# lainy/sdrangel

Measured on AMD Instinct MI355X. Metric: MS/s complex int16 IQ through decim-64 + DownChannelizer, 1/2/4/8 GPU; % HBM roofline, higher is better.
Workload: dtype int32

## Files before the change

sdrangel_amd/csrc/chan_lower.cpp:

```cpp
#include "chan_lower.hpp"
#include "chan_plan.hpp"
#include <algorithm>

namespace sdrx {

bool subtree_all_mx(const TkSubtree& st)
{
    if (st.n_levels < 1 || st.n_levels > MX_MAX_LEVELS) return false;
    for (int l = 0; l < st.n_levels; l++) if (!st.lv[l].mfma) return false;
    return true;
}

namespace {

std::string lower_job(const TkMJob& j, int PI, int PO, TkLJob& r)
{
    r.b = j.bI; r.c = j.mode ? j.cQ : j.cI; r.out0 = j.out0;
    if (j.bQ != j.bI + PI) return "lower: odd arms not one pitch apart";
    if ((j.mode ? j.cI - j.cQ : j.cQ - j.cI) != PI) return "lower: even arms not one pitch apart";
    bool sink = false;
    int meta = 0;
    for (int k = 0; k < 2; k++) {
        const TkMOut& m = j.o[k];
        const int f = m.flags;
        r.sink[k] = m.sink;
        sink |= m.sink >= 0;
        if (f != 0 && f != (1 | 2) && f != (1 | 4) && f != (1 | 2 | 4)) return "lower: unexpected arm set";
        r.o[k] = f ? m.E_I : 0;
        if (f) {
            if (m.E_Q != m.E_I + PO) return "lower: even arms of a child not one pitch apart";
            const int odd_I = (f & 2) || j.fast ? m.O_I : m.A_I, odd_Q = (f & 2) || j.fast ? m.O_Q : m.A_Q;
            if (odd_I != m.E_I + 2 * PO || odd_Q != m.E_I + 3 * PO) return "lower: odd arm of a child not at 2 pitches";
            if (f == 7 && (m.A_I != m.E_I + 4 * PO || m.A_Q != m.E_I + 5 * PO)) return "lower: alternating arm of a child not at 4 pitches";
        }
        meta |= f << (4 + 4 * k);
    }
    if (!j.mode && (j.o[1].flags || j.o[1].sink >= 0)) return "lower: centre stage with a second child";
    if (j.fast && sink) return "lower: branch-free job with a sink";
    const int cls = j.fast ? MX_FAST : sink ? MX_SINK : MX_ARMS;
    if (j.mode) meta |= MX_LU_BIT;
    r.meta = meta | cls;
    return {};
}

std::string lower_subtree(const BankPlan& plan, const TkSubtree& st, LoweredBank& out)
{
    std::string err;
    for (int l = 0; l < st.n_levels; l++) {
        const TkLevel& lv = st.lv[l];
        const int PI = mx_pitch(l), PO = mx_pitch(l + 1);
        if (lv.in_len * 4 != PI || (lv.arr_cnt && lv.arr_len * 4 != PO)) return "lower: level arrays of another length";
        std::vector<std::pair<int, int>> order;
        std::vector<TkLJob> lowered((size_t)lv.n_mjobs);
        for (int q = 0; q < lv.n_mjobs; q++) {
            const int i = lv.mjob_base + q;
            err = lower_job(plan.mjobs[(size_t)i], PI, PO, lowered[(size_t)q]);
            if (!err.empty()) return err;
            order.emplace_back(mx_class(lowered[(size_t)q].meta), q);
        }
        std::stable_sort(order.begin(), order.end(), [](const std::pair<int, int>& a, const std::pair<int, int>& b) { return a.first < b.first; });
        for (int q = 0; q < lv.n_mjobs; q++) {
            out.jobs[(size_t)(lv.mjob_base + q)] = lowered[(size_t)order[(size_t)q].second];
            out.src[(size_t)(lv.mjob_base + q)] = lv.mjob_base + order[(size_t)q].second;
        }
    }
    return {};
}

}

std::string lower_bank(const BankPlan& plan, LoweredBank& out)
{
    out = LoweredBank{};
    out.jobs.resize(plan.mjobs.size());
    out.src.resize(plan.mjobs.size());
    for (size_t i = 0; i < plan.mjobs.size(); i++) out.src[i] = (int)i;
    std::string first_err;
    std::vector<uint8_t> sub_mx(plan.subtrees.size(), 0);
    for (size_t s = 0; s < plan.subtrees.size(); s++) {
        const TkSubtree& st = plan.subtrees[s];
        if (!plan.mfma || !subtree_all_mx(st)) continue;
        const std::string err = lower_subtree(plan, st, out);
        if (err.empty()) sub_mx[s] = 1;
        else if (first_err.empty()) first_err = err;
    }
    out.pass_mx.assign(plan.passes.size(), 0);
    for (size_t p = 0; p < plan.passes.size(); p++) {
        bool all = !plan.passes[p].empty();
        for (int si : plan.passes[p]) {
            const int s = plan.streams[(size_t)si].subtree;
            all = all && s >= 0 && sub_mx[(size_t)s];
        }
        out.pass_mx[p] = plan.mfma && all ? 1 : 0;
    }
    return first_err;
}

}
```

sdrangel_amd/csrc/chan_lower.hpp:

```cpp
#pragma once
#include "tree_layout.hpp"
#include "hb_consts.hpp"
#include <string>
#include <vector>

namespace sdrx {

struct BankPlan;

constexpr int MX_MAX_LEVELS = 4;

constexpr int mx_pitch(int rel) { return 4 * (HIST / 2 + (TK_CHUNK >> (rel + 2))); }

enum : int {
    MX_FAST = 0,
    MX_ARMS = 1,
    MX_SINK = 2,
    MX_CLASSES = 3
};
constexpr int MX_LU_BIT = 1 << 16;

struct TkLJob {
    int b;
    int c;
    int o[2];
    int sink[2];
    int out0;
    int meta;
};
static_assert(sizeof(TkLJob) == 32, "one s_load_dwordx8 per job");

inline int mx_class(int meta) { return meta & 15; }
inline int mx_flags(int meta, int k) { return (meta >> (4 + 4 * k)) & 15; }

struct LoweredBank {
    std::vector<TkLJob> jobs;
    std::vector<int> src;
    std::vector<uint8_t> pass_mx;
};

bool subtree_all_mx(const TkSubtree& st);

std::string lower_bank(const BankPlan& plan, LoweredBank& out);

}
```

sdrangel_amd/csrc/sdrx_chan.hip:

```cpp
#include "sdrx_common.hpp"
#include "chan_plan.hpp"
#include "tree_kernel.hpp"
#include "tree_mx_kernel.hpp"
#include <vector>
#include <cstring>
#include <new>
#include <algorithm>
#include "chan_plan.cpp"
#include "chan_lower.cpp"

using namespace sdrx;

namespace {

struct Channel {
    int32_t out_rate = 0, ofs = 0;
    int n = 0;
    uint8_t modes[32] = { 0 };
    int group = -1;
    bool passthrough = false;
    bool dead = false;
    DevBuf out;
    int64_t avail = 0;
    int64_t last_off = 0, last_n = 0;
};

struct StreamBuf {
    uint32_t* hist[2] = { nullptr, nullptr };
    int cur = 0;
    DevBuf mid;
};

struct Group {
    int index = -1;
    int64_t T = 0;
    std::vector<int> chans;
    BankPlan plan;
    LoweredBank low;
    std::vector<StreamBuf> bufs;
    void* d_static = nullptr;
    TkSubtree* d_subtrees = nullptr; TkNode* d_nodes = nullptr; TkArray* d_arrays = nullptr; TkMJob* d_mjobs = nullptr;
    TkLJob* d_ljobs = nullptr;
};

}

struct sdrx_chan_bank {
    int device = 0, cus = 256;
    int32_t in_rate = 0;
    hipStream_t own_stream = nullptr, stream = nullptr;
    std::vector<Channel> ch;
    std::vector<Group*> groups;
    DevBuf stage_in;
    DevBuf scratch;
    static constexpr int RING = 4;
    void* h_dyn[RING] = { nullptr, nullptr, nullptr, nullptr };
    void* d_dyn[RING] = { nullptr, nullptr, nullptr, nullptr };
    size_t dyn_cap[RING] = { 0, 0, 0, 0 };
    hipEvent_t dyn_ev[RING] = { nullptr, nullptr, nullptr, nullptr };
    int dyn_next = 0;
    char last_name[96] = "";
    int last_grid = 0, last_block = 0, last_lds = 0;
    EventTimer timer;
};

static void free_group(Group* g)
{
    if (!g) return;
    for (auto& s : g->bufs) { for (uint32_t* h : s.hist) if (h) (void)hipFree(h); s.mid.release(); }
    if (g->d_static) (void)hipFree(g->d_static);
    delete g;
}

static int upload_group(sdrx_chan_bank* b, Group* g)
{
    const BankPlan& p = g->plan;
    g->bufs.resize(p.streams.size());
    for (size_t si = 0; si < p.streams.size(); si++) {
        const size_t bytes = (size_t)p.streams[si].hist_len * 4;
        for (uint32_t*& h : g->bufs[si].hist) {
            SDRX_HIP(hipMalloc(reinterpret_cast<void**>(&h), bytes));
            SDRX_HIP(hipMemsetAsync(h, 0, bytes, b->stream));
        }
    }
    const size_t b0 = p.subtrees.size() * sizeof(TkSubtree), b1 = p.nodes.size() * sizeof(TkNode), b2 = p.arrays.size() * sizeof(TkArray);
    const size_t b3 = p.mjobs.size() * sizeof(TkMJob), b4 = g->low.jobs.size() * sizeof(TkLJob);
    if (b0 + b1 + b2 == 0) return SDRX_OK;
    SDRX_HIP(hipMalloc(&g->d_static, b0 + b1 + b2 + b3 + b4 + 64));
    char* d = static_cast<char*>(g->d_static);
    g->d_subtrees = reinterpret_cast<TkSubtree*>(d);
    g->d_nodes = reinterpret_cast<TkNode*>(d + b0);
    g->d_arrays = reinterpret_cast<TkArray*>(d + b0 + b1);
    g->d_mjobs = reinterpret_cast<TkMJob*>(d + b0 + b1 + b2);
    g->d_ljobs = reinterpret_cast<TkLJob*>(d + b0 + b1 + b2 + b3);
    if (b0) SDRX_HIP(hipMemcpy(g->d_subtrees, p.subtrees.data(), b0, hipMemcpyHostToDevice));
    if (b1) SDRX_HIP(hipMemcpy(g->d_nodes, p.nodes.data(), b1, hipMemcpyHostToDevice));
    if (b2) SDRX_HIP(hipMemcpy(g->d_arrays, p.arrays.data(), b2, hipMemcpyHostToDevice));
    if (b3) SDRX_HIP(hipMemcpy(g->d_mjobs, p.mjobs.data(), b3, hipMemcpyHostToDevice));
    if (b4) SDRX_HIP(hipMemcpy(g->d_ljobs, g->low.jobs.data(), b4, hipMemcpyHostToDevice));
    return SDRX_OK;
}

static int configure_channel(sdrx_chan_bank* b, int c, int32_t req_rate, int32_t req_fc)
{
    Channel& ch = b->ch[c];
    ch.n = plan_chain(b->in_rate, req_rate, req_fc, ch.modes, MAX_STAGES, &ch.out_rate, &ch.ofs);
    ch.passthrough = ch.n == 0;
    return SDRX_OK;
}

static int new_group(sdrx_chan_bank* b, const std::vector<int>& chans)
{
    if (chans.empty()) return SDRX_OK;
    std::vector<PlanChain> chains;
    for (int c : chans) chains.push_back(PlanChain{ c, b->ch[(size_t)c].n, b->ch[(size_t)c].modes });
    BankPlan plan;
    const std::string err = plan_bank(chains, plan_options_from_env(), plan);
    if (!err.empty()) { set_error(err); return SDRX_EINVAL; }
    LoweredBank low;
    (void)lower_bank(plan, low);
    Group* g = new (std::nothrow) Group;
    if (!g) return SDRX_ENOMEM;
    g->chans = chans;
    g->index = (int)b->groups.size();
    g->plan = std::move(plan);
    g->low = std::move(low);
    int rc = upload_group(b, g);
    if (rc) { free_group(g); return rc; }
    for (int c : chans) b->ch[c].group = g->index;
    b->groups.push_back(g);
    return SDRX_OK;
}

static int retire_dead_groups(sdrx_chan_bank* b)
{
    for (size_t gi = 0; gi < b->groups.size();) {
        Group* g = b->groups[gi];
        bool live = false;
        for (int c : g->chans) if (b->ch[(size_t)c].group == g->index) { live = true; break; }
        if (live) { gi++; continue; }
        SDRX_HIP(hipStreamSynchronize(b->stream));
        free_group(g);
        b->groups.erase(b->groups.begin() + (long)gi);
        for (size_t k = gi; k < b->groups.size(); k++) {
            const int old = b->groups[k]->index;
            b->groups[k]->index = (int)k;
            for (int c : b->groups[k]->chans) if (b->ch[(size_t)c].group == old) b->ch[(size_t)c].group = (int)k;
        }
    }
    return SDRX_OK;
}

static int grow_keep(sdrx_chan_bank* b, DevBuf& buf, size_t used, size_t need)
{
    if (need <= buf.cap) return SDRX_OK;
    size_t want = buf.cap ? buf.cap : (1 << 16);
    while (want < need) want *= 2;
    void* np = nullptr;
    SDRX_HIP(hipMalloc(&np, want));
    if (used) SDRX_HIP(hipMemcpyAsync(np, buf.p, used, hipMemcpyDeviceToDevice, b->stream));
    SDRX_HIP(hipStreamSynchronize(b->stream));
    if (buf.p) (void)hipFree(buf.p);
    buf.p = np; buf.cap = want;
    return SDRX_OK;
}

static int dyn_slot(sdrx_chan_bank* b, size_t bytes, int* slot)
{
    const int s = b->dyn_next; b->dyn_next = (b->dyn_next + 1) % sdrx_chan_bank::RING;
    if (b->dyn_ev[s]) SDRX_HIP(hipEventSynchronize(b->dyn_ev[s]));
    else SDRX_HIP(hipEventCreateWithFlags(&b->dyn_ev[s], hipEventDisableTiming));
    if (bytes > b->dyn_cap[s]) {
        size_t want = b->dyn_cap[s] ? b->dyn_cap[s] : 4096; while (want < bytes) want *= 2;
        if (b->h_dyn[s]) (void)hipHostFree(b->h_dyn[s]);
        if (b->d_dyn[s]) (void)hipFree(b->d_dyn[s]);
        b->h_dyn[s] = b->d_dyn[s] = nullptr; b->dyn_cap[s] = 0;
        SDRX_HIP(hipHostMalloc(&b->h_dyn[s], want, hipHostMallocDefault));
        SDRX_HIP(hipMalloc(&b->d_dyn[s], want));
        b->dyn_cap[s] = want;
    }
    *slot = s;
    return SDRX_OK;
}

static int feed_group(sdrx_chan_bank* b, Group* g, const uint32_t* d_in, int64_t n)
{
    const int64_t T0 = g->T, T1 = g->T + n;
    for (int c : g->chans) {
        Channel& ch = b->ch[c];
        if (ch.group != g->index) continue;
        const int64_t add = (T1 >> ch.n) - (T0 >> ch.n);
        int rc = grow_keep(b, ch.out, (size_t)ch.avail * 4, (size_t)(ch.avail + add) * 4 + 64); if (rc) return rc;
    }
    const BankPlan& plan = g->plan;
    for (size_t si = 1; si < plan.streams.size(); si++) {
        const int64_t add = (T1 >> plan.streams[si].depth) - (T0 >> plan.streams[si].depth);
        int rc = g->bufs[si].mid.reserve((size_t)add * 4 + 64); if (rc) return rc;
    }
    const size_t ns = plan.streams.size(), nk = plan.sinks.size();
    const size_t o_sinks = ns * sizeof(TkStream), o_hist = o_sinks + nk * sizeof(TkSink), total = o_hist + ns * sizeof(TkHistJob);
    int slot; int rc = dyn_slot(b, total, &slot); if (rc) return rc;
    char* hp = static_cast<char*>(b->h_dyn[slot]); char* dp = static_cast<char*>(b->d_dyn[slot]);
    TkStream* hs = reinterpret_cast<TkStream*>(hp);
    TkSink* hk = reinterpret_cast<TkSink*>(hp + o_sinks);
    TkHistJob* hh = reinterpret_cast<TkHistJob*>(hp + o_hist);

    std::vector<long> segs(ns, 0);
    for (size_t si = 0; si < ns; si++) {
        const PlanStream& s = plan.streams[si];
        const StreamBuf& sb = g->bufs[si];
        TkStream& t = hs[si];
        t.hist = sb.hist[sb.cur];
        t.in = si == 0 ? d_in : static_cast<const uint32_t*>(sb.mid.p);
        t.t_old = T0 >> s.depth; t.t_new = T1 >> s.depth;
        t.subtree = s.subtree;
        t.c_first = t.t_old / TK_CHUNK;
        t.c_last = t.t_new > t.t_old ? (t.t_new - 1) / TK_CHUNK : t.c_first - 1;
        t.cps = 1;
        t.hist_len = s.hist_len;
        hh[si] = TkHistJob{ sb.hist[sb.cur], t.in, sb.hist[sb.cur ^ 1], t.t_new - t.t_old, s.hist_len };
    }
    for (size_t k = 0; k < nk; k++) {
        const PlanSink& si = plan.sinks[k];
        TkSink& t = hk[k];
        t.shift = 0; t.next = si.next;
        if (si.kind == 0) {
            Channel& ch = b->ch[si.ch];
            t.lo = T0 >> si.depth; t.hi = T1 >> si.depth;
            t.ptr0 = reinterpret_cast<uint32_t*>(reinterpret_cast<uintptr_t>(ch.out.p) - (uintptr_t)(4 * (t.lo - ch.avail)));
            t.shift = si.depth;
            if (ch.group != g->index) t.hi = t.lo;
        } else {
            const int depth = plan.streams[(size_t)si.stream].depth;
            t.lo = T0 >> depth; t.hi = T1 >> depth;
            t.ptr0 = reinterpret_cast<uint32_t*>(reinterpret_cast<uintptr_t>(g->bufs[(size_t)si.stream].mid.p) - (uintptr_t)(4 * t.lo));
        }
    }
    for (const std::vector<int>& ps : plan.passes) {
        long total_chunks = 0;
        for (int si : ps) total_chunks += std::max(0L, hs[si].c_last - hs[si].c_first + 1);
        long cps = (total_chunks + (long)b->cus * 4 - 1) / ((long)b->cus * 4);
        cps = std::max(1L, std::min(cps, 256L));
        for (int si : ps) {
            hs[si].cps = (int)cps;
            segs[si] = (std::max(0L, hs[si].c_last - hs[si].c_first + 1) + cps - 1) / cps;
        }
    }
    SDRX_HIP(hipMemcpyAsync(dp, hp, total, hipMemcpyHostToDevice, b->stream));
    SDRX_HIP(hipEventRecord(b->dyn_ev[slot], b->stream));

    const TkStream* d_streams = reinterpret_cast<const TkStream*>(dp);
    const TkSink* d_sinks = reinterpret_cast<const TkSink*>(dp + o_sinks);
    const TkHistJob* d_hist = reinterpret_cast<const TkHistJob*>(dp + o_hist);
    rc = b->timer.begin(b->stream); if (rc) return rc;
    for (size_t p = 0; p < plan.passes.size(); p++) {
        const std::vector<int>& ps = plan.passes[p];
        if (ps.empty()) continue;
        long max_segs = 0;
        for (int si : ps) max_segs = std::max(max_segs, segs[si]);
        if (max_segs == 0) continue;
        const int s0 = ps.front(), cnt = (int)ps.size();
        size_t lds_bytes = 0;
        for (int si : ps) lds_bytes = std::max(lds_bytes, (size_t)plan.subtrees[(size_t)plan.streams[(size_t)si].subtree].lds_dwords * 4);
        if (g->low.pass_mx[p])
            hipLaunchKernelGGL(tree_mx_kernel, dim3((unsigned)max_segs, (unsigned)cnt), dim3(TK_THREADS), lds_bytes, b->stream,
                               g->d_subtrees, g->d_arrays, d_streams + s0, d_sinks, g->d_ljobs);
        else if (plan.mfma)
            hipLaunchKernelGGL(tree_kernel<true>, dim3((unsigned)max_segs, (unsigned)cnt), dim3(TK_THREADS), lds_bytes, b->stream,
                               g->d_subtrees, g->d_nodes, g->d_arrays, d_streams + s0, d_sinks, g->d_mjobs);
        else
            hipLaunchKernelGGL(tree_kernel<false>, dim3((unsigned)max_segs, (unsigned)cnt), dim3(TK_THREADS), lds_bytes, b->stream,
                               g->d_subtrees, g->d_nodes, g->d_arrays, d_streams + s0, d_sinks, g->d_mjobs);
        SDRX_HIP(hipGetLastError());
        if (p == 0) {
            snprintf(b->last_name, sizeof b->last_name, plan.mfma ? "tree_kernel<mfma>" : "tree_kernel<valu>");
            b->last_grid = (int)(max_segs * cnt); b->last_block = TK_THREADS; b->last_lds = (int)lds_bytes;
        }
    }
    rc = b->timer.end(b->stream); if (rc) return rc;
    long max_hist = TK_HIST;
    for (const PlanStream& s : plan.streams) max_hist = std::max(max_hist, s.hist_len);
    hipLaunchKernelGGL(tree_hist_kernel, dim3((unsigned)(max_hist / 256), (unsigned)ns), dim3(256), 0, b->stream, d_hist);
    SDRX_HIP(hipGetLastError());
    for (StreamBuf& sb : g->bufs) sb.cur ^= 1;
    for (int c : g->chans) {
        Channel& ch = b->ch[c];
        if (ch.group != g->index) continue;
        const int64_t add = (T1 >> ch.n) - (T0 >> ch.n);
        ch.last_off = ch.avail; ch.last_n = add; ch.avail += add;
    }
    g->T = T1;
    return SDRX_OK;
}

static int feed_passthrough(sdrx_chan_bank* b, const uint32_t* d_in, int64_t n)
{
    for (auto& ch : b->ch) {
        if (!ch.passthrough) continue;
        int rc = grow_keep(b, ch.out, (size_t)ch.avail * 4, (size_t)(ch.avail + n) * 4 + 64); if (rc) return rc;
        SDRX_HIP(hipMemcpyAsync(static_cast<uint32_t*>(ch.out.p) + ch.avail, d_in, (size_t)n * 4, hipMemcpyDeviceToDevice, b->stream));
        ch.last_off = ch.avail; ch.last_n = n; ch.avail += n;
    }
    return SDRX_OK;
}

extern "C" {

int sdrx_chan_plan(int32_t in_rate, int32_t req_rate, int32_t req_fc, uint8_t* modes, int32_t* out_rate, int32_t* residual_ofs)
{
    if (!modes || !out_rate || !residual_ofs) { set_error("sdrx_chan_plan: null argument"); return SDRX_EINVAL; }
    return plan_chain(in_rate, req_rate, req_fc, modes, MAX_STAGES, out_rate, residual_ofs);
}

int sdrx_chan_bank_create(sdrx_chan_bank_t** out, int device, int32_t in_rate, int32_t n_ch,
                          const int32_t* req_rate, const int32_t* req_fc)
{
    if (!out) { set_error("sdrx_chan_bank_create: null out"); return SDRX_EINVAL; }
    *out = nullptr;
    if (n_ch <= 0 || !req_rate || !req_fc || in_rate <= 0) { set_error("sdrx_chan_bank_create: bad argument"); return SDRX_EINVAL; }
    int rc = check_device(device); if (rc) return rc;
    SDRX_HIP(hipSetDevice(device));
    sdrx_chan_bank* b = new (std::nothrow) sdrx_chan_bank;
    if (!b) return SDRX_ENOMEM;
    b->device = device; b->in_rate = in_rate; b->cus = device_cu_count(device);
    hipError_t e = hipStreamCreateWithFlags(&b->own_stream, hipStreamNonBlocking);
    if (e != hipSuccess) { delete b; return hip_fail(e, "hipStreamCreate", __FILE__, __LINE__); }
    b->stream = b->own_stream;
    e = hipFuncSetAttribute(reinterpret_cast<const void*>(&tree_kernel<true>), hipFuncAttributeMaxDynamicSharedMemorySize, 160 * 1024);
    if (e == hipSuccess) e = hipFuncSetAttribute(reinterpret_cast<const void*>(&tree_kernel<false>), hipFuncAttributeMaxDynamicSharedMemorySize, 160 * 1024);
    if (e == hipSuccess) e = hipFuncSetAttribute(reinterpret_cast<const void*>(&tree_mx_kernel), hipFuncAttributeMaxDynamicSharedMemorySize, 160 * 1024);
    if (e != hipSuccess) { sdrx_chan_bank_destroy(b); return hip_fail(e, "hipFuncSetAttribute", __FILE__, __LINE__); }
    b->ch.resize((size_t)n_ch);
    std::vector<int> all;
    for (int c = 0; c < n_ch; c++) {
        configure_channel(b, c, req_rate[c], req_fc[c]);
        if (!b->ch[c].passthrough) all.push_back(c);
    }
    rc = new_group(b, all);
    if (rc) { sdrx_chan_bank_destroy(b); return rc; }
    SDRX_HIP(hipStreamSynchronize(b->stream));
    *out = b;
    return SDRX_OK;
}

int sdrx_chan_bank_destroy(sdrx_chan_bank_t* b)
{
    if (!b) return SDRX_OK;
    (void)hipSetDevice(b->device);
    if (b->stream) (void)hipStreamSynchronize(b->stream);
    for (Group* g : b->groups) free_group(g);
    for (auto& c : b->ch) c.out.release();
    b->stage_in.release(); b->scratch.release(); b->timer.release();
    for (int i = 0; i < sdrx_chan_bank::RING; i++) {
        if (b->h_dyn[i]) (void)hipHostFree(b->h_dyn[i]);
        if (b->d_dyn[i]) (void)hipFree(b->d_dyn[i]);
        if (b->dyn_ev[i]) (void)hipEventDestroy(b->dyn_ev[i]);
    }
    if (b->own_stream) (void)hipStreamDestroy(b->own_stream);
    delete b;
    return SDRX_OK;
}

int sdrx_chan_bank_info(const sdrx_chan_bank_t* b, int32_t c, int32_t* n_stages, uint8_t* modes, int32_t* out_rate, int32_t* residual_ofs)
{
    if (!b || c < 0 || c >= (int32_t)b->ch.size()) { set_error("sdrx_chan_bank_info: bad channel"); return SDRX_EINVAL; }
    const Channel& ch = b->ch[(size_t)c];
    if (n_stages) *n_stages = ch.n;
    if (modes) memcpy(modes, ch.modes, (size_t)ch.n);
    if (out_rate) *out_rate = ch.out_rate;
    if (residual_ofs) *residual_ofs = ch.ofs;
    return SDRX_OK;
}

int sdrx_chan_bank_reconfigure(sdrx_chan_bank_t* b, int32_t c, int32_t req_rate, int32_t req_fc)
{
    if (!b || c < 0 || c >= (int32_t)b->ch.size()) { set_error("sdrx_chan_bank_reconfigure: bad channel"); return SDRX_EINVAL; }
    SDRX_HIP(hipSetDevice(b->device));
    Channel& ch = b->ch[(size_t)c];
    ch.group = -1; ch.dead = false;
    configure_channel(b, c, req_rate, req_fc);
    int rc = retire_dead_groups(b); if (rc) return rc;
    if (ch.passthrough) return SDRX_OK;
    return new_group(b, std::vector<int>{ (int)c });
}

int sdrx_chan_bank_add_channel(sdrx_chan_bank_t* b, int32_t req_rate, int32_t req_fc, int32_t* channel)
{
    if (!b) { set_error("sdrx_chan_bank_add_channel: null bank"); return SDRX_EINVAL; }
    SDRX_HIP(hipSetDevice(b->device));
    b->ch.emplace_back();
    const int c = (int)b->ch.size() - 1;
    configure_channel(b, c, req_rate, req_fc);
    if (channel) *channel = c;
    if (b->ch[(size_t)c].passthrough) return SDRX_OK;
    const int rc = new_group(b, std::vector<int>{ c });
    if (rc) { b->ch.pop_back(); if (channel) *channel = -1; }
    return rc;
}

int sdrx_chan_bank_remove_channel(sdrx_chan_bank_t* b, int32_t c)
{
    if (!b || c < 0 || c >= (int32_t)b->ch.size()) { set_error("sdrx_chan_bank_remove_channel: bad channel"); return SDRX_EINVAL; }
    SDRX_HIP(hipSetDevice(b->device));
    Channel& ch = b->ch[(size_t)c];
    ch.group = -1; ch.passthrough = false; ch.dead = true; ch.n = 0; ch.out_rate = 0; ch.ofs = 0;
    ch.avail = 0; ch.last_off = 0; ch.last_n = 0;
    return retire_dead_groups(b);
}

static const int64_t CHAN_STATE_MAGIC = 0x7364727863686b31LL;

int64_t sdrx_chan_bank_state_bytes(const sdrx_chan_bank_t* b)
{
    if (!b) return SDRX_EINVAL;
    int64_t n = 16;
    for (const Group* g : b->groups) { n += 16; for (const PlanStream& s : g->plan.streams) n += 8 + (int64_t)s.hist_len * 4; }
    return n;
}

// ... 199 lines not shown
```

sdrangel_amd/csrc/tree_mx_kernel.hpp:

```cpp
#pragma once
#include "hb_common.hpp"
#include "hb_mfma.hpp"
#include "tree_layout.hpp"
#include "chan_lower.hpp"

namespace sdrx {

__device__ __forceinline__ int mx_div_pow2_trunc(int v, int n)
{
    return (v + ((v >> 31) & ((1 << n) - 1))) >> n;
}

__global__ __launch_bounds__(TK_THREADS, 4)
void tree_mx_kernel(const TkSubtree* __restrict__ subtrees, const TkArray* __restrict__ arrays, const TkStream* __restrict__ streams,
                    const TkSink* __restrict__ sinks, const TkLJob* __restrict__ ljobs)
{
    constexpr int C = TK_CHUNK, NT = TK_THREADS, LPT = C / 4 / NT;
    extern __shared__ __attribute__((aligned(16))) uint32_t lds[];

    const TkStream sp = streams[blockIdx.y];
    const long first = sp.c_first + (long)blockIdx.x * sp.cps;
    if (first > sp.c_last) return;
    long last = first + sp.cps - 1; if (last > sp.c_last) last = sp.c_last;
    const TkSubtree& st = subtrees[sp.subtree];
    const int tid = threadIdx.x;

    for (int i = tid; i < st.lds_dwords; i += NT) lds[i] = 0;
    __syncthreads();
    for (int i = tid; i < st.n_arrays * 16; i += NT) {
        const TkArray a = arrays[st.array_base + (i >> 4)];
        if (a.bias) lds[a.store + (i & 15)] = HBM_BIAS2;
    }
    typedef HbMfmaTaps<48, false> Taps;
    Taps taps;
    const int lane = tid & 63, n16 = lane & 15, g4 = lane >> 4;
    const int wv = __builtin_amdgcn_readfirstlane(tid >> 6);
    taps.init(lane);
    const uint32_t root_xm = st.root_xm;
    int n_levels = st.n_levels, store_base = st.store_base, root_off = st.root_off, root_len = st.root_len;
    asm volatile("" : "+s"(n_levels), "+s"(store_base), "+s"(root_off), "+s"(root_len));
    int rE_I = st.rootE_I, rE_Q = st.rootE_Q, rO_I = st.rootO_I, rO_Q = st.rootO_Q, rA_I = st.rootA_I, rA_Q = st.rootA_Q, root_cnt16 = st.root_arr_cnt * 16;
    asm volatile("" : "+s"(rE_I), "+s"(rE_Q), "+s"(rO_I), "+s"(rO_Q), "+s"(rA_I), "+s"(rA_Q), "+s"(root_cnt16));

    uint4 pre[LPT];
    auto fetch = [&](long chunk, const int tid) {
        const long c0 = chunk * C;
        if (c0 >= sp.t_old && c0 + C <= sp.t_new) {
            typedef uint32_t u4v __attribute__((ext_vector_type(4)));
            typedef const u4v __attribute__((address_space(1))) gq4;
            gq4* src = (gq4*)reinterpret_cast<const u4v*>(sp.in + (c0 - sp.t_old));
#pragma unroll
            for (int j = 0; j < LPT; j++) { const u4v v = src[j * NT + tid]; pre[j] = make_uint4(v[0], v[1], v[2], v[3]); }
            return;
        }
#pragma unroll
        for (int j = 0; j < LPT; j++) {
            const long p0 = chunk * C + 4 * (j * NT + tid);
            if (p0 >= sp.t_old && p0 + 4 <= sp.t_new) {
                pre[j] = *reinterpret_cast<const uint4*>(sp.in + (p0 - sp.t_old));
            } else {
                uint32_t v[4];
#pragma unroll
                for (int e = 0; e < 4; e++) {
                    const long p = p0 + e;
                    v[e] = p < sp.t_old ? sp.hist[p - (sp.t_old - sp.hist_len)] : (p < sp.t_new ? sp.in[p - sp.t_old] : 0u);
                }
                pre[j] = make_uint4(v[0], v[1], v[2], v[3]);
            }
        }
        __builtin_amdgcn_s_waitcnt(0x0F70);
    };
    fetch(first - st.warm, tid);
    __syncthreads();

    typedef int s8i __attribute__((ext_vector_type(8)));
    typedef int s16i __attribute__((ext_vector_type(16)));
    typedef unsigned short us2 __attribute__((ext_vector_type(2)));
    const v4i bias = { Taps::BIAS, Taps::BIAS, Taps::BIAS, Taps::BIAS };
    const char* ldsb = reinterpret_cast<const char*>(lds);
    char* ldsw = reinterpret_cast<char*>(lds);
    const int wl = 32 * n16 + 16 * g4, cl = 32 * n16 + 8 * g4, pl = 16 * n16 + 4 * g4;
    constexpr uint32_t PLAIN = 0x00010001u, ALT = 0x0001ffffu;
    auto padd = [](uint32_t a, uint32_t b) { return __builtin_bit_cast(uint32_t, (us2)(__builtin_bit_cast(us2, a) + __builtin_bit_cast(us2, b))); };
    auto psub = [](uint32_t a, uint32_t b) { return __builtin_bit_cast(uint32_t, (us2)(__builtin_bit_cast(us2, a) - __builtin_bit_cast(us2, b))); };
    auto pmul = [](uint32_t a, uint32_t m) { return __builtin_bit_cast(uint32_t, (us2)(__builtin_bit_cast(us2, a) * __builtin_bit_cast(us2, m))); };

    for (long chunk = first - st.warm; chunk <= last; ++chunk) {
        int tid = threadIdx.x;
        asm volatile("" : "+v"(tid));
#pragma unroll
        for (int j = 0; j < LPT; j++) {
            const int q = HIST / 2 + j * NT + tid;
            const uint4 v = pre[j];
            const uint32_t oI = __builtin_amdgcn_perm(v.w, v.y, 0x05040100u);
            const uint32_t oQ = __builtin_amdgcn_perm(v.w, v.y, 0x07060302u);
            lds[rE_I + q] = __builtin_amdgcn_perm(v.z, v.x, 0x05040100u);
            lds[rE_Q + q] = __builtin_amdgcn_perm(v.z, v.x, 0x07060302u);
            if (rO_I >= 0) { lds[rO_I + q] = oI ^ root_xm; lds[rO_Q + q] = oQ ^ root_xm; }
            if (rA_I >= 0) { lds[rA_I + q] = pmul(oI, ALT) ^ root_xm; lds[rA_Q + q] = pmul(oQ, ALT) ^ root_xm; }
        }
        for (int i = tid; i < root_cnt16; i += NT)
            lds[root_off + (i >> 4) * root_len + (i & 15)] = lds[store_base + i];
        if (chunk < last) fetch(chunk + 1, tid);
        __syncthreads();

        const bool live = chunk >= first;
        int lv0 = 0;
        asm volatile("" : "+s"(lv0), "+s"(n_levels));
        auto level = [&](auto Lc) {
            constexpr int L = decltype(Lc)::value;
            constexpr int PI = mx_pitch(L), PO = mx_pitch(L + 1);
            const s16i rec = *(const s16i __attribute__((address_space(4)))*)reinterpret_cast<const int*>(&st.lv[L + lv0]);
            const int nout = rec[3], arr_base = rec[4], arr_cnt = rec[5], in_len = rec[7], mjob_base = rec[9], n_mjobs = rec[10];
            const uint32_t xm = (uint32_t)rec[11];
            const int prev_off = rec[12], prev_arr_cnt = rec[13], arr_off = rec[14], arr_len = rec[15];
            {
                const int n_restore = arr_cnt * 16, n_all = n_restore + prev_arr_cnt * 16;
                const int slot0 = store_base + 16 * arr_base;
                for (int i = tid; i < n_all; i += NT) {
                    const int k = i - n_restore;
                    const int src = k < 0 ? slot0 + i : prev_off + (k >> 4) * in_len + in_len - 16 + (k & 15);
                    const int dst = k < 0 ? arr_off + (i >> 4) * arr_len + (i & 15) : slot0 - prev_arr_cnt * 16 + k;
                    lds[dst] = lds[src];
                }
            }
            struct JobIn { v4i bI0, bI1, bQ0, bQ1; uint2 cI01, cQ01; uint32_t cI2, cQ2; };
            auto load = [&](const s8i d, JobIn& r, auto Cc) {
                const char* pb = ldsb + d[0] + wl;
                r.bI0 = *reinterpret_cast<const v4i*>(__builtin_assume_aligned(pb, 16));
                r.bI1 = *reinterpret_cast<const v4i*>(__builtin_assume_aligned(pb + 64, 16));
                r.bQ0 = *reinterpret_cast<const v4i*>(__builtin_assume_aligned(pb + PI, 16));
                r.bQ1 = *reinterpret_cast<const v4i*>(__builtin_assume_aligned(pb + PI + 64, 16));
                const char* pc = ldsb + d[1] + cl;
                const char *pI, *pQ;
                if constexpr (decltype(Cc)::value == MX_FAST) { pI = pc + PI; pQ = pc; }
                else { const bool lu = d[7] & MX_LU_BIT; pI = lu ? pc + PI : pc; pQ = lu ? pc : pc + PI; }
                r.cI01 = *reinterpret_cast<const uint2*>(__builtin_assume_aligned(pI, 8));
                r.cI2 = *reinterpret_cast<const uint32_t*>(pI + 8);
                r.cQ01 = *reinterpret_cast<const uint2*>(__builtin_assume_aligned(pQ, 8));
                r.cQ2 = *reinterpret_cast<const uint32_t*>(pQ + 8);
            };
            auto st32 = [&](char* p, int off, uint32_t v) { *reinterpret_cast<uint32_t*>(p + off) = v; };
            auto child = [&](auto Sk, const uint32_t eI, const uint32_t oI, const uint32_t eQ, const uint32_t oQ, const int base, const int f,
                             const int sink, const long abs0) {
                constexpr bool SINK = decltype(Sk)::value;
                if (f) {
                    char* p = ldsw + base + pl;
                    const uint32_t m = (f & 2) ? PLAIN : ALT;
                    st32(p, 0, eI); st32(p, PO, eQ);
                    st32(p, 2 * PO, pmul(oI, m) ^ xm); st32(p, 3 * PO, pmul(oQ, m) ^ xm);
                    if (f == 7) { st32(p, 4 * PO, pmul(oI, ALT) ^ xm); st32(p, 5 * PO, pmul(oQ, ALT) ^ xm); }
                }
                if constexpr (SINK) {
                    if (live) {
                        typedef const s8i __attribute__((address_space(4))) cs8;
                        for (int si = sink; si >= 0; ) {
                            const s8i sr = *(cs8*)reinterpret_cast<const int*>(sinks + si);
                            const long ptr0 = ((long)sr[1] << 32) | (uint32_t)sr[0];
                            const long lo = ((long)sr[3] << 32) | (uint32_t)sr[2], hi = ((long)sr[5] << 32) | (uint32_t)sr[4];
                            const int shift = sr[6];
                            uint32_t w[4];
                            if (shift) {
                                w[0] = pack_iq(mx_div_pow2_trunc((int)(int16_t)eI, shift), mx_div_pow2_trunc((int)(int16_t)eQ, shift));
                                w[1] = pack_iq(mx_div_pow2_trunc((int)(int16_t)oI, shift), mx_div_pow2_trunc((int)(int16_t)oQ, shift));
                                w[2] = pack_iq(mx_div_pow2_trunc((int)eI >> 16, shift), mx_div_pow2_trunc((int)eQ >> 16, shift));
                                w[3] = pack_iq(mx_div_pow2_trunc((int)oI >> 16, shift), mx_div_pow2_trunc((int)oQ >> 16, shift));
                            } else {
                                w[0] = __builtin_amdgcn_perm(eQ, eI, 0x05040100u); w[1] = __builtin_amdgcn_perm(oQ, oI, 0x05040100u);
                                w[2] = __builtin_amdgcn_perm(eQ, eI, 0x07060302u); w[3] = __builtin_amdgcn_perm(oQ, oI, 0x07060302u);
                            }
                            typedef uint32_t __attribute__((address_space(1))) gu32;
                            gu32* dst = (gu32*)(reinterpret_cast<uint32_t*>(ptr0) + abs0);
                            const long rel = abs0 - lo, span = hi - lo;
                            if (rel >= 0 && rel + 4 <= span) {
                                typedef uint32_t u4a __attribute__((ext_vector_type(4), aligned(4)));
                                *(u4a __attribute__((address_space(1)))*)dst = u4a{ w[0], w[1], w[2], w[3] };
                            } else if (rel > -4 && rel < span) {
#pragma unroll
                                for (int i = 0; i < 4; i++) if (rel + i >= 0 && rel + i < span) dst[i] = w[i];
                            }
                            si = sr[7];
                        }
                    }
                }
            };
            auto finish = [&](auto Cc, const JobIn& r, const v4i SI, const v4i SQ, const s8i d) {
                constexpr int CLS = decltype(Cc)::value;
                auto shpack = [](int a, int b) {
                    uint32_t v = (uint32_t)(a >> (HB_SHIFT - 1));
                    asm("v_ashrrev_i32_sdwa %0, %1, %2 dst_sel:WORD_1 dst_unused:UNUSED_PRESERVE src0_sel:DWORD src1_sel:DWORD" : "+v"(v) : "s"(HB_SHIFT - 1), "v"(b));
                    return v;
                };
                const uint32_t sI02 = shpack(SI[0], SI[2]), sI13 = shpack(SI[1], SI[3]);
                const uint32_t sQ02 = shpack(SQ[0], SQ[2]), sQ13 = shpack(SQ[1], SQ[3]);
                const uint32_t cI02 = __builtin_amdgcn_perm(r.cI01.y, r.cI01.x, 0x07060302u), cI13 = __builtin_amdgcn_perm(r.cI2, r.cI01.y, 0x05040100u);
                const uint32_t cQ02 = __builtin_amdgcn_perm(r.cQ01.y, r.cQ01.x, 0x07060302u), cQ13 = __builtin_amdgcn_perm(r.cQ2, r.cQ01.y, 0x05040100u);
                const int meta = d[7], f0 = (meta >> 4) & 15, f1 = (meta >> 8) & 15;
                if constexpr (CLS == MX_FAST) {
                    const uint32_t ma = (f0 & 2) ? PLAIN : ALT, mb = (f1 & 2) ? PLAIN : ALT;
                    auto st4 = [&](const int base, uint32_t eI, uint32_t eQ, uint32_t oI, uint32_t oQ, uint32_t m) {
                        char* p = ldsw + base + pl;
                        st32(p, 0, eI); st32(p, PO, eQ); st32(p, 2 * PO, pmul(oI, m) ^ xm); st32(p, 3 * PO, pmul(oQ, m) ^ xm);
                    };
                    st4(d[2], padd(sI02, cI02), psub(sQ02, cQ02), psub(sI13, cI13), padd(sQ13, cQ13), ma);
                    st4(d[3], psub(sI02, cI02), padd(sQ02, cQ02), padd(sI13, cI13), psub(sQ13, cQ13), mb);
                } else {
                    const std::integral_constant<bool, CLS == MX_SINK> Sk;
                    const long abs0 = CLS == MX_SINK ? chunk * nout + d[6] + 16 * n16 + 4 * g4 : 0;
                    const uint32_t sg = (meta & MX_LU_BIT) ? 0xffffffffu : PLAIN;
                    if (f0 | (d[4] >= 0)) {
                        const uint32_t nI13 = pmul(cI13, sg), nQ02 = pmul(cQ02, sg);
                        child(Sk, padd(sI02, cI02), padd(sI13, nI13), padd(sQ02, nQ02), padd(sQ13, cQ13), d[2], f0, d[4], abs0);
                    }
                    if (f1 | (d[5] >= 0)) child(Sk, psub(sI02, cI02), padd(sI13, cI13), padd(sQ02, cQ02), psub(sQ13, cQ13), d[3], f1, d[5], abs0);
                }
            };
            auto pair = [&](auto Cc, const s8i d0, const s8i d1) {
                JobIn r0, r1;
                __builtin_amdgcn_s_setprio(2);
                load(d0, r0, Cc); load(d1, r1, Cc);
                __builtin_amdgcn_sched_barrier(0);
                const v4i SI0 = taps.tile(r0.bI0, r0.bI1, bias), SQ0 = taps.tile(r0.bQ0, r0.bQ1, bias);
                const v4i SI1 = taps.tile(r1.bI0, r1.bI1, bias), SQ1 = taps.tile(r1.bQ0, r1.bQ1, bias);
                __builtin_amdgcn_s_setprio(0);
                finish(Cc, r0, SI0, SQ0, d0);
                finish(Cc, r1, SI1, SQ1, d1);
            };
            auto single = [&](auto Cc, const s8i d0) {
                JobIn r0;
                load(d0, r0, Cc);
                const v4i SI0 = taps.tile(r0.bI0, r0.bI1, bias), SQ0 = taps.tile(r0.bQ0, r0.bQ1, bias);
                finish(Cc, r0, SI0, SQ0, d0);
            };
            typedef std::integral_constant<int, MX_FAST> KF;
            typedef std::integral_constant<int, MX_ARMS> KA;
            typedef std::integral_constant<int, MX_SINK> KS;
            const int per = (n_mjobs + NT / 64 - 1) / (NT / 64);
            const int t0 = wv * per, t1 = t0 + per < n_mjobs ? t0 + per : n_mjobs;
            typedef const s8i __attribute__((address_space(4))) cs8j;
            for (int tt = t0; tt < t1; ) {
                const s8i d0 = *(cs8j*)reinterpret_cast<const int*>(ljobs + mjob_base + tt);
                const int c0 = d0[7] & 15;
                if (tt + 1 < t1) {
                    const s8i d1 = *(cs8j*)reinterpret_cast<const int*>(ljobs + mjob_base + tt + 1);
                    if ((d1[7] & 15) == c0) {
                        if (c0 == MX_FAST) pair(KF{}, d0, d1);
                        else if (c0 == MX_ARMS) pair(KA{}, d0, d1);
                        else pair(KS{}, d0, d1);
                        tt += 2;
                        continue;
                    }
                }
                if (c0 == MX_FAST) single(KF{}, d0);
                else if (c0 == MX_ARMS) single(KA{}, d0);
                else single(KS{}, d0);
                tt += 1;
            }
            __syncthreads();
        };
        level(std::integral_constant<int, 0>{});
        if (n_levels > 1) level(std::integral_constant<int, 1>{});
        if (n_levels > 2) level(std::integral_constant<int, 2>{});
        if (n_levels > 3) level(std::integral_constant<int, 3>{});
    }
}

}
```

Measured before the change: 252,700.

## Precompile per-wave job step programs with scalar prefetch of next step

The host lowering now emits a linear per-wave program for each subtree: a 64-byte level-header step, then single or pair job steps with kind and end flags packed into meta bits. The MX kernel walks this program and issues the scalar load for the next step while the current job's MFMA work runs. This replaces per-level record reads, per-wave range arithmetic and pairwise class checks. Level sizes become compile-time constants (guarded by a new lowering check), and sink stores gain a branch-light in-range fast path. The cost is extra host-side program memory and more complex control and waitcnt handling in the kernel.

```diff
diff --git a/sdrangel_amd/csrc/chan_lower.cpp b/sdrangel_amd/csrc/chan_lower.cpp
--- a/sdrangel_amd/csrc/chan_lower.cpp
+++ b/sdrangel_amd/csrc/chan_lower.cpp
@@ -50,6 +50,7 @@
         const TkLevel& lv = st.lv[l];
         const int PI = mx_pitch(l), PO = mx_pitch(l + 1);
         if (lv.in_len * 4 != PI || (lv.arr_cnt && lv.arr_len * 4 != PO)) return "lower: level arrays of another length";
+        if (lv.nout != TK_CHUNK >> (l + 1)) return "lower: level outputs of another count";
         std::vector<std::pair<int, int>> order;
         std::vector<TkLJob> lowered((size_t)lv.n_mjobs);
         for (int q = 0; q < lv.n_mjobs; q++) {
@@ -67,6 +68,34 @@
     return {};
 }
 
+void emit_programs(const TkSubtree& st, int subtree, LoweredBank& out)
+{
+    for (int w = 0; w < MX_WAVES; w++) {
+        out.prog_index[(size_t)(subtree * MX_WAVES + w)] = (int)out.prog.size();
+        for (int l = 0; l < st.n_levels; l++) {
+            const TkLevel& lv = st.lv[l];
+            TkStep s{};
+            s.w[0] = lv.arr_base; s.w[1] = lv.arr_cnt; s.w[2] = lv.prev_off; s.w[3] = lv.prev_arr_cnt; s.w[4] = lv.arr_off; s.w[5] = (int)lv.xm;
+            s.w[7] = MX_STEP_LEVEL << MX_STEP_KIND_SHIFT;
+            out.prog.push_back(s);
+            const int per = (lv.n_mjobs + MX_WAVES - 1) / MX_WAVES;
+            const int t0 = w * per, t1 = std::min(t0 + per, lv.n_mjobs);
+            for (int t = t0; t < t1; ) {
+                const TkLJob* j = &out.jobs[(size_t)(lv.mjob_base + t)];
+                const bool two = t + 1 < t1 && mx_class(j[1].meta) == mx_class(j[0].meta);
+                TkStep js{};
+                static_assert(sizeof(TkLJob) == 8 * sizeof(int), "a job is half a step");
+                const int* src = reinterpret_cast<const int*>(j);
+                std::copy(src, src + (two ? 16 : 8), js.w);
+                js.w[7] |= (two ? MX_STEP_PAIR : MX_STEP_SINGLE) << MX_STEP_KIND_SHIFT;
+                out.prog.push_back(js);
+                t += two ? 2 : 1;
+            }
+            out.prog.back().w[7] |= MX_STEP_END_LEVEL | (l == st.n_levels - 1 ? MX_STEP_END_CHUNK : 0);
+        }
+    }
+}
+
 }
 
 std::string lower_bank(const BankPlan& plan, LoweredBank& out)
@@ -77,13 +106,15 @@
     for (size_t i = 0; i < plan.mjobs.size(); i++) out.src[i] = (int)i;
     std::string first_err;
     std::vector<uint8_t> sub_mx(plan.subtrees.size(), 0);
+    out.prog_index.assign(plan.subtrees.size() * MX_WAVES, -1);
     for (size_t s = 0; s < plan.subtrees.size(); s++) {
         const TkSubtree& st = plan.subtrees[s];
         if (!plan.mfma || !subtree_all_mx(st)) continue;
         const std::string err = lower_subtree(plan, st, out);
-        if (err.empty()) sub_mx[s] = 1;
+        if (err.empty()) { sub_mx[s] = 1; emit_programs(st, (int)s, out); }
         else if (first_err.empty()) first_err = err;
     }
+    out.prog.push_back(TkStep{});
     out.pass_mx.assign(plan.passes.size(), 0);
     for (size_t p = 0; p < plan.passes.size(); p++) {
         bool all = !plan.passes[p].empty();
diff --git a/sdrangel_amd/csrc/chan_lower.hpp b/sdrangel_amd/csrc/chan_lower.hpp
--- a/sdrangel_amd/csrc/chan_lower.hpp
+++ b/sdrangel_amd/csrc/chan_lower.hpp
@@ -33,10 +33,22 @@
 inline int mx_class(int meta) { return meta & 15; }
 inline int mx_flags(int meta, int k) { return (meta >> (4 + 4 * k)) & 15; }
 
+enum : int { MX_STEP_PAD = 0, MX_STEP_LEVEL = 1, MX_STEP_SINGLE = 2, MX_STEP_PAIR = 3 };
+constexpr int MX_STEP_KIND_SHIFT = 17;
+constexpr int MX_STEP_END_LEVEL = 1 << 20, MX_STEP_END_CHUNK = 1 << 21;
+constexpr int MX_JOB_META_MASK = (1 << MX_STEP_KIND_SHIFT) - 1;
+constexpr int MX_WAVES = TK_THREADS / 64;
+struct alignas(64) TkStep { int w[16]; };
+static_assert(sizeof(TkStep) == 64, "one s_load_dwordx16 per step");
+
+constexpr int mx_step_kind(int bits) { return (bits >> MX_STEP_KIND_SHIFT) & 3; }
+
 struct LoweredBank {
     std::vector<TkLJob> jobs;
     std::vector<int> src;
     std::vector<uint8_t> pass_mx;
+    std::vector<TkStep> prog;
+    std::vector<int> prog_index;
 };
 
 bool subtree_all_mx(const TkSubtree& st);
diff --git a/sdrangel_amd/csrc/sdrx_chan.hip b/sdrangel_amd/csrc/sdrx_chan.hip
--- a/sdrangel_amd/csrc/sdrx_chan.hip
+++ b/sdrangel_amd/csrc/sdrx_chan.hip
@@ -40,7 +40,7 @@
     std::vector<StreamBuf> bufs;
     void* d_static = nullptr;
     TkSubtree* d_subtrees = nullptr; TkNode* d_nodes = nullptr; TkArray* d_arrays = nullptr; TkMJob* d_mjobs = nullptr;
-    TkLJob* d_ljobs = nullptr;
+    TkStep* d_prog = nullptr; int* d_prog_index = nullptr;
 };
 
 }
@@ -84,20 +84,23 @@
         }
     }
     const size_t b0 = p.subtrees.size() * sizeof(TkSubtree), b1 = p.nodes.size() * sizeof(TkNode), b2 = p.arrays.size() * sizeof(TkArray);
-    const size_t b3 = p.mjobs.size() * sizeof(TkMJob), b4 = g->low.jobs.size() * sizeof(TkLJob);
+    const size_t b3 = p.mjobs.size() * sizeof(TkMJob), b4 = g->low.prog.size() * sizeof(TkStep), b5 = g->low.prog_index.size() * sizeof(int);
+    const size_t o4 = (b0 + b1 + b2 + b3 + 63) / 64 * 64;
     if (b0 + b1 + b2 == 0) return SDRX_OK;
-    SDRX_HIP(hipMalloc(&g->d_static, b0 + b1 + b2 + b3 + b4 + 64));
+    SDRX_HIP(hipMalloc(&g->d_static, o4 + b4 + b5 + 64));
     char* d = static_cast<char*>(g->d_static);
     g->d_subtrees = reinterpret_cast<TkSubtree*>(d);
     g->d_nodes = reinterpret_cast<TkNode*>(d + b0);
     g->d_arrays = reinterpret_cast<TkArray*>(d + b0 + b1);
     g->d_mjobs = reinterpret_cast<TkMJob*>(d + b0 + b1 + b2);
-    g->d_ljobs = reinterpret_cast<TkLJob*>(d + b0 + b1 + b2 + b3);
+    g->d_prog = reinterpret_cast<TkStep*>(d + o4);
+    g->d_prog_index = reinterpret_cast<int*>(d + o4 + b4);
     if (b0) SDRX_HIP(hipMemcpy(g->d_subtrees, p.subtrees.data(), b0, hipMemcpyHostToDevice));
     if (b1) SDRX_HIP(hipMemcpy(g->d_nodes, p.nodes.data(), b1, hipMemcpyHostToDevice));
     if (b2) SDRX_HIP(hipMemcpy(g->d_arrays, p.arrays.data(), b2, hipMemcpyHostToDevice));
     if (b3) SDRX_HIP(hipMemcpy(g->d_mjobs, p.mjobs.data(), b3, hipMemcpyHostToDevice));
-    if (b4) SDRX_HIP(hipMemcpy(g->d_ljobs, g->low.jobs.data(), b4, hipMemcpyHostToDevice));
+    if (b4) SDRX_HIP(hipMemcpy(g->d_prog, g->low.prog.data(), b4, hipMemcpyHostToDevice));
+    if (b5) SDRX_HIP(hipMemcpy(g->d_prog_index, g->low.prog_index.data(), b5, hipMemcpyHostToDevice));
     return SDRX_OK;
 }
 
@@ -264,7 +267,7 @@
         for (int si : ps) lds_bytes = std::max(lds_bytes, (size_t)plan.subtrees[(size_t)plan.streams[(size_t)si].subtree].lds_dwords * 4);
         if (g->low.pass_mx[p])
             hipLaunchKernelGGL(tree_mx_kernel, dim3((unsigned)max_segs, (unsigned)cnt), dim3(TK_THREADS), lds_bytes, b->stream,
-                               g->d_subtrees, g->d_arrays, d_streams + s0, d_sinks, g->d_ljobs);
+                               g->d_subtrees, g->d_arrays, d_streams + s0, d_sinks, g->d_prog, g->d_prog_index);
         else if (plan.mfma)
             hipLaunchKernelGGL(tree_kernel<true>, dim3((unsigned)max_segs, (unsigned)cnt), dim3(TK_THREADS), lds_bytes, b->stream,
                                g->d_subtrees, g->d_nodes, g->d_arrays, d_streams + s0, d_sinks, g->d_mjobs);
diff --git a/sdrangel_amd/csrc/tree_mx_kernel.hpp b/sdrangel_amd/csrc/tree_mx_kernel.hpp
--- a/sdrangel_amd/csrc/tree_mx_kernel.hpp
+++ b/sdrangel_amd/csrc/tree_mx_kernel.hpp
@@ -13,7 +13,7 @@
 
 __global__ __launch_bounds__(TK_THREADS, 4)
 void tree_mx_kernel(const TkSubtree* __restrict__ subtrees, const TkArray* __restrict__ arrays, const TkStream* __restrict__ streams,
-                    const TkSink* __restrict__ sinks, const TkLJob* __restrict__ ljobs)
+                    const TkSink* __restrict__ sinks, const TkStep* __restrict__ prog, const int* __restrict__ prog_index)
 {
     constexpr int C = TK_CHUNK, NT = TK_THREADS, LPT = C / 4 / NT;
     extern __shared__ __attribute__((aligned(16))) uint32_t lds[];
@@ -36,6 +36,16 @@
     const int lane = tid & 63, n16 = lane & 15, g4 = lane >> 4;
     const int wv = __builtin_amdgcn_readfirstlane(tid >> 6);
     taps.init(lane);
+    typedef int s16i __attribute__((ext_vector_type(16)));
+    typedef const s16i __attribute__((address_space(4))) cs16;
+    const TkStep* const prog0 = prog + prog_index[sp.subtree * MX_WAVES + wv];
+    const TkStep* pc = prog0;
+    s16i step;
+    auto request = [&](const TkStep* at) {
+        __builtin_amdgcn_sched_barrier(0);
+        step = *(cs16*)reinterpret_cast<const int*>(at);
+        __builtin_amdgcn_sched_barrier(0);
+    };
     const uint32_t root_xm = st.root_xm;
     int n_levels = st.n_levels, store_base = st.store_base, root_off = st.root_off, root_len = st.root_len;
     asm volatile("" : "+s"(n_levels), "+s"(store_base), "+s"(root_off), "+s"(root_len));
@@ -74,9 +84,9 @@
     __syncthreads();
 
     typedef int s8i __attribute__((ext_vector_type(8)));
-    typedef int s16i __attribute__((ext_vector_type(16)));
     typedef unsigned short us2 __attribute__((ext_vector_type(2)));
-    const v4i bias = { Taps::BIAS, Taps::BIAS, Taps::BIAS, Taps::BIAS };
+    v4i bias = { Taps::BIAS, Taps::BIAS, Taps::BIAS, Taps::BIAS };
+    asm volatile("" : "+v"(bias));
     const char* ldsb = reinterpret_cast<const char*>(lds);
     char* ldsw = reinterpret_cast<char*>(lds);
     const int wl = 32 * n16 + 16 * g4, cl = 32 * n16 + 8 * g4, pl = 16 * n16 + 4 * g4;
@@ -88,6 +98,9 @@
     for (long chunk = first - st.warm; chunk <= last; ++chunk) {
         int tid = threadIdx.x;
         asm volatile("" : "+v"(tid));
+        pc = prog0;
+        asm volatile("" : "+s"(pc));
+        request(pc);
 #pragma unroll
         for (int j = 0; j < LPT; j++) {
             const int q = HIST / 2 + j * NT + tid;
@@ -105,15 +118,15 @@
         __syncthreads();
 
         const bool live = chunk >= first;
-        int lv0 = 0;
-        asm volatile("" : "+s"(lv0), "+s"(n_levels));
+        asm volatile("" : "+s"(n_levels));
         auto level = [&](auto Lc) {
             constexpr int L = decltype(Lc)::value;
             constexpr int PI = mx_pitch(L), PO = mx_pitch(L + 1);
-            const s16i rec = *(const s16i __attribute__((address_space(4)))*)reinterpret_cast<const int*>(&st.lv[L + lv0]);
-            const int nout = rec[3], arr_base = rec[4], arr_cnt = rec[5], in_len = rec[7], mjob_base = rec[9], n_mjobs = rec[10];
-            const uint32_t xm = (uint32_t)rec[11];
-            const int prev_off = rec[12], prev_arr_cnt = rec[13], arr_off = rec[14], arr_len = rec[15];
+            constexpr int nout = C >> (L + 1), in_len = PI / 4, arr_len = PO / 4;
+            const s16i rec = step;
+            request(++pc);
+            const int arr_base = rec[0], arr_cnt = rec[1], prev_off = rec[2], prev_arr_cnt = rec[3], arr_off = rec[4];
+            const uint32_t xm = (uint32_t)rec[5];
             {
                 const int n_restore = arr_cnt * 16, n_all = n_restore + prev_arr_cnt * 16;
                 const int slot0 = store_base + 16 * arr_base;
@@ -142,7 +155,7 @@
             };
             auto st32 = [&](char* p, int off, uint32_t v) { *reinterpret_cast<uint32_t*>(p + off) = v; };
             auto child = [&](auto Sk, const uint32_t eI, const uint32_t oI, const uint32_t eQ, const uint32_t oQ, const int base, const int f,
-                             const int sink, const long abs0) {
+                             const int sink, const long job0) {
                 constexpr bool SINK = decltype(Sk)::value;
                 if (f) {
                     char* p = ldsw + base + pl;
@@ -170,14 +183,22 @@
                                 w[2] = __builtin_amdgcn_perm(eQ, eI, 0x07060302u); w[3] = __builtin_amdgcn_perm(oQ, oI, 0x07060302u);
                             }
                             typedef uint32_t __attribute__((address_space(1))) gu32;
-                            gu32* dst = (gu32*)(reinterpret_cast<uint32_t*>(ptr0) + abs0);
-                            const long rel = abs0 - lo, span = hi - lo;
-                            if (rel >= 0 && rel + 4 <= span) {
-                                typedef uint32_t u4a __attribute__((ext_vector_type(4), aligned(4)));
+                            typedef uint32_t u4a __attribute__((ext_vector_type(4), aligned(4)));
+                            int in_feed = (int)((unsigned long)((job0 - lo) | (hi - 256 - job0)) >> 32);
+                            asm("" : "+s"(in_feed));
+                            if (__builtin_expect(in_feed >= 0, 1)) {
+                                gu32* dst = (gu32*)(reinterpret_cast<char*>(ptr0) + job0 * 4 + (uint32_t)(4 * pl));
                                 *(u4a __attribute__((address_space(1)))*)dst = u4a{ w[0], w[1], w[2], w[3] };
-                            } else if (rel > -4 && rel < span) {
-#pragma unroll
-                                for (int i = 0; i < 4; i++) if (rel + i >= 0 && rel + i < span) dst[i] = w[i];
+                            } else {
+                                const long abs0 = job0 + pl;
+                                gu32* dst = (gu32*)(reinterpret_cast<uint32_t*>(ptr0) + abs0);
+                                const long rel = abs0 - lo, span = hi - lo;
+                                if (rel >= 0 && rel + 4 <= span) {
+                                    *(u4a __attribute__((address_space(1)))*)dst = u4a{ w[0], w[1], w[2], w[3] };
+                                } else if (rel > -4 && rel < span) {
+#pragma unroll
+                                    for (int i = 0; i < 4; i++) if (rel + i >= 0 && rel + i < span) dst[i] = w[i];
+                                }
                             }
                             si = sr[7];
                         }
@@ -206,55 +227,60 @@
                     st4(d[3], psub(sI02, cI02), padd(sQ02, cQ02), padd(sI13, cI13), psub(sQ13, cQ13), mb);
                 } else {
                     const std::integral_constant<bool, CLS == MX_SINK> Sk;
-                    const long abs0 = CLS == MX_SINK ? chunk * nout + d[6] + 16 * n16 + 4 * g4 : 0;
+                    const long job0 = CLS == MX_SINK ? chunk * nout + d[6] : 0;
                     const uint32_t sg = (meta & MX_LU_BIT) ? 0xffffffffu : PLAIN;
                     if (f0 | (d[4] >= 0)) {
                         const uint32_t nI13 = pmul(cI13, sg), nQ02 = pmul(cQ02, sg);
-                        child(Sk, padd(sI02, cI02), padd(sI13, nI13), padd(sQ02, nQ02), padd(sQ13, cQ13), d[2], f0, d[4], abs0);
+                        child(Sk, padd(sI02, cI02), padd(sI13, nI13), padd(sQ02, nQ02), padd(sQ13, cQ13), d[2], f0, d[4], job0);
                     }
-                    if (f1 | (d[5] >= 0)) child(Sk, psub(sI02, cI02), padd(sI13, cI13), padd(sQ02, cQ02), psub(sQ13, cQ13), d[3], f1, d[5], abs0);
-                }
+                    if (f1 | (d[5] >= 0)) child(Sk, psub(sI02, cI02), padd(sI13, cI13), padd(sQ02, cQ02), psub(sQ13, cQ13), d[3], f1, d[5], job0);
+                }
+            };
+            auto landed = [](JobIn& r) { asm volatile("" : "+v"(r.cI01.x), "+v"(r.cI01.y), "+v"(r.cI2), "+v"(r.cQ01.x), "+v"(r.cQ01.y), "+v"(r.cQ2)); };
+            auto body = [](auto Id) {
+                asm volatile("; job body %0" :: "n"(decltype(Id)::value) : "memory");
+                __builtin_amdgcn_s_waitcnt(0xC07F);
             };
             auto pair = [&](auto Cc, const s8i d0, const s8i d1) {
                 JobIn r0, r1;
+                body(std::integral_constant<int, 2 * decltype(Cc)::value + 1>{});
                 __builtin_amdgcn_s_setprio(2);
                 load(d0, r0, Cc); load(d1, r1, Cc);
                 __builtin_amdgcn_sched_barrier(0);
                 const v4i SI0 = taps.tile(r0.bI0, r0.bI1, bias), SQ0 = taps.tile(r0.bQ0, r0.bQ1, bias);
                 const v4i SI1 = taps.tile(r1.bI0, r1.bI1, bias), SQ1 = taps.tile(r1.bQ0, r1.bQ1, bias);
                 __builtin_amdgcn_s_setprio(0);
+                landed(r0); landed(r1);
+                request(++pc);
                 finish(Cc, r0, SI0, SQ0, d0);
                 finish(Cc, r1, SI1, SQ1, d1);
             };
             auto single = [&](auto Cc, const s8i d0) {
                 JobIn r0;
+                body(std::integral_constant<int, 2 * decltype(Cc)::value>{});
                 load(d0, r0, Cc);
                 const v4i SI0 = taps.tile(r0.bI0, r0.bI1, bias), SQ0 = taps.tile(r0.bQ0, r0.bQ1, bias);
+                landed(r0);
+                request(++pc);
                 finish(Cc, r0, SI0, SQ0, d0);
             };
             typedef std::integral_constant<int, MX_FAST> KF;
             typedef std::integral_constant<int, MX_ARMS> KA;
             typedef std::integral_constant<int, MX_SINK> KS;
-            const int per = (n_mjobs + NT / 64 - 1) / (NT / 64);
-            const int t0 = wv * per, t1 = t0 + per < n_mjobs ? t0 + per : n_mjobs;
-            typedef const s8i __attribute__((address_space(4))) cs8j;
-            for (int tt = t0; tt < t1; ) {
-                const s8i d0 = *(cs8j*)reinterpret_cast<const int*>(ljobs + mjob_base + tt);
-                const int c0 = d0[7] & 15;
-                if (tt + 1 < t1) {
-                    const s8i d1 = *(cs8j*)reinterpret_cast<const int*>(ljobs + mjob_base + tt + 1);
-                    if ((d1[7] & 15) == c0) {
-                        if (c0 == MX_FAST) pair(KF{}, d0, d1);
-                        else if (c0 == MX_ARMS) pair(KA{}, d0, d1);
-                        else pair(KS{}, d0, d1);
-                        tt += 2;
-                        continue;
-                    }
-                }
-                if (c0 == MX_FAST) single(KF{}, d0);
-                else if (c0 == MX_ARMS) single(KA{}, d0);
-                else single(KS{}, d0);
-                tt += 1;
+            for (int bits = rec[7]; !(bits & MX_STEP_END_LEVEL); ) {
+                const s16i cur = step;
+                bits = cur[7];
+                const s8i d0 = __builtin_shufflevector(cur, cur, 0, 1, 2, 3, 4, 5, 6, 7), d1 = __builtin_shufflevector(cur, cur, 8, 9, 10, 11, 12, 13, 14, 15);
+                const int c0 = bits & 15;
+                if (mx_step_kind(bits) == MX_STEP_PAIR) {
+                    if (c0 == MX_FAST) pair(KF{}, d0, d1);
+                    else if (c0 == MX_ARMS) pair(KA{}, d0, d1);
+                    else pair(KS{}, d0, d1);
+                } else {
+                    if (c0 == MX_FAST) single(KF{}, d0);
+                    else if (c0 == MX_ARMS) single(KA{}, d0);
+                    else single(KS{}, d0);
+                }
             }
             __syncthreads();
         };
```

After: 258,300, median of 6. 2.2% higher.
